# PKU-EPIC/GAPartNet

Hardware: AMD Instinct MI355X
Metric: point-clouds/sec (20k pts, train step) (higher is better)
Workload: dtype f32

## Files before the change

gapartnet_amd/csrc/bn.hip:

```cpp
#include <cstdlib>

#include "bn_stats.h"
#include "gpn_common.h"

namespace {

typedef float f32x4 __attribute__((ext_vector_type(4)));
constexpr int kThreads = 256;
constexpr int kMaxBlocks = 128;


template <int T>
__device__ __forceinline__ double column_total(const double (*red)[T][4], int q, int c, int C4, int R, int part, int P) {
  double acc = 0.0;
  const int cc4 = c >> 2, j = c & 3;
  for (int rr = part; rr < R; rr += P) acc += red[q][rr * C4 + cc4][j];
  for (int off = P >> 1; off >= 1; off >>= 1) acc += __shfl_down(acc, off, P);
  return acc;
}

__host__ __device__ __forceinline__ int sub_lanes(int pairs, int T) {
  int P = 16;
  while (P > 1 && pairs * P > T) P >>= 1;
  return P;
// ... 302 lines not shown
        if (res) v += rv[k];
        if (relu) {
#pragma unroll
          for (int j = 0; j < 4; ++j) v[j] = v[j] > 0.f ? v[j] : 0.f;
        }
        reinterpret_cast<f32x4*>(y)[tt] = v;
      }
      c4 += step;
      c4 = c4 >= C4 ? c4 - C4 : c4;
    }
    t += U * stride;
    if (t >= total4) break;
#pragma unroll
    for (int k = 0; k < U; ++k) {
      const int64_t tt = t + k * stride;
      if (tt < total4) {
        xv[k] = reinterpret_cast<const f32x4*>(x)[tt];
        if (res) rv[k] = reinterpret_cast<const f32x4*>(res)[tt];
      }
    }
  }
}

template <bool FIXED>
__global__ __launch_bounds__(kApplyThreads) void bn_apply_bwd_fold_kernel(gpn::BnBwdPtrs pa, gpn::BnBwdPtrs pb, int blocks, int64_t total4,
                                                                         int C4, float inv_n, int relu, int training,
                                                                         const int64_t* __restrict__ n_dev) {
  if (n_dev) {
    const int64_t N = gpn::live_rows(n_dev, total4 / C4);
    total4 = N * C4;
    inv_n = 1.0f / (float)N;
    if (N == 0) {
      if (blockIdx.x == 0) {
        const gpn::BnBwdPtrs& q = blockIdx.y ? pb : pa;
        for (int c = threadIdx.x; c < C4 * 4; c += kApplyThreads) q.dbias[c] = 0.f, q.dweight[c] = 0.f;
      }
      return;
    }
  }
  const gpn::BnBwdPtrs& pp = blockIdx.y ? pb : pa;
  const float* __restrict__ x = pp.x;
  const float* __restrict__ y = pp.y;
  const float* __restrict__ dy = pp.dy;
  const void* __restrict__ partial = pp.partial;
  const float* __restrict__ mean = pp.mean;
  const float* __restrict__ invstd = pp.invstd;
  const float* __restrict__ weight = pp.weight;
  float* __restrict__ dx = pp.dx;
  float* __restrict__ dres = pp.dres;
  float* __restrict__ dweight = pp.dweight;
  float* __restrict__ dbias = pp.dbias;
  __shared__ double red[2][FIXED ? 1 : kApplyThreads][4];
  __shared__ unsigned long long words[FIXED ? 4 : 1][FIXED ? kFoldMaxC : 1];
  __shared__ double sums[2][kFoldMaxC];
  __shared__ __attribute__((aligned(16))) float stat[5][kFoldMaxC];
  constexpr int U = kApplyBatch;
  const int C = C4 * 4;
  const int64_t stride = (int64_t)gridDim.x * kApplyThreads;
  const int step = (int)(stride % C4);
  int64_t t = (int64_t)blockIdx.x * kApplyThreads + threadIdx.x;
  int c4 = (int)(t % C4);
  f32x4 gv[U], yv[U], xv[U];
#pragma unroll
  for (int k = 0; k < U; ++k) {
    const int64_t tt = t + k * stride;
    if (tt < total4) {
      gv[k] = reinterpret_cast<const f32x4*>(dy)[tt];
      if (relu) yv[k] = reinterpret_cast<const f32x4*>(y)[tt];
      if (training) xv[k] = reinterpret_cast<const f32x4*>(x)[tt];
    }
  }
  if constexpr (FIXED)
    fold_fixed<true>(static_cast<const unsigned long long*>(partial), C, blocks, reinterpret_cast<unsigned long long (*)[kFoldMaxC]>(&words[0][0]), sums);
  else
    fold_partials(static_cast<const double*>(partial), blocks, C4, reinterpret_cast<double (*)[kApplyThreads][4]>(&red[0][0][0]), sums);
  for (int c = threadIdx.x; c < C; c += kApplyThreads) {
    const float db = (float)sums[0][c], dw = (float)sums[1][c];
    stat[0][c] = db;
    stat[1][c] = dw;
    stat[2][c] = mean[c];
    stat[3][c] = invstd[c];
    stat[4][c] = weight[c];
    if (blockIdx.x == 0) {
      dbias[c] = db;
      dweight[c] = dw;
    }
  }
  __syncthreads();
  while (true) {
#pragma unroll
    for (int k = 0; k < U; ++k) {
      const int64_t tt = t + k * stride;
      if (tt < total4) {
        const f32x4 is = reinterpret_cast<const f32x4*>(stat[3])[c4], w = reinterpret_cast<const f32x4*>(stat[4])[c4];
        f32x4 g = gv[k];
        if (relu) {
#pragma unroll
          for (int j = 0; j < 4; ++j) g[j] = yv[k][j] > 0.f ? g[j] : 0.f;
        }
        if (dres) reinterpret_cast<f32x4*>(dres)[tt] = g;
        f32x4 v = g;
        if (training) {
          const f32x4 db = reinterpret_cast<const f32x4*>(stat[0])[c4], dw = reinterpret_cast<const f32x4*>(stat[1])[c4];
          const f32x4 mu = reinterpret_cast<const f32x4*>(stat[2])[c4];
          const f32x4 xhat = (xv[k] - mu) * is;
          v = g - db * inv_n - xhat * (dw * inv_n);
        }
        reinterpret_cast<f32x4*>(dx)[tt] = v * is * w;
      }
      c4 += step;
      c4 = c4 >= C4 ? c4 - C4 : c4;
    }
    t += U * stride;
    if (t >= total4) break;
#pragma unroll
    for (int k = 0; k < U; ++k) {
      const int64_t tt = t + k * stride;
      if (tt < total4) {
        gv[k] = reinterpret_cast<const f32x4*>(dy)[tt];
        if (relu) yv[k] = reinterpret_cast<const f32x4*>(y)[tt];
        if (training) xv[k] = reinterpret_cast<const f32x4*>(x)[tt];
      }
    }
  }
}

constexpr int kSmallRows = 1024;

template <int CG, int T>
__device__ __forceinline__ void column_sum8(double (&v)[8], double (*scratch)[CG][8] ) {
  constexpr int W = T / 64;
#pragma unroll
  for (int off = 32; off >= CG; off >>= 1) {
#pragma unroll
    for (int q = 0; q < 8; ++q) v[q] += __shfl_down(v[q], off, 64);
  }
  if ((threadIdx.x & 63) < CG) {
#pragma unroll
    for (int q = 0; q < 8; ++q) scratch[threadIdx.x >> 6][threadIdx.x & 63][q] = v[q];
  }
  __syncthreads();
  const int cg = threadIdx.x % CG;
#pragma unroll
// ... 302 lines not shown
}

bool gpn::bn_two_pass(int64_t N, int C) { return N >= 1 && C % 4 == 0 && C <= kFoldMaxC; }

int gpn::bn_fwd_train_fused(const gpn::BnFwdPtrs& p, const gpn::BnFwdPtrs* twin, int64_t N, int C, float eps, float momentum,
                            int relu, hipStream_t stream, const gpn::DevRows& rows) {
  for (const gpn::BnFwdPtrs* q : {&p, twin}) {
    if (!q) continue;
    GPN_CHECK_ARG(q->x && q->weight && q->bias && q->y && q->mean && q->invstd && q->partial);
    GPN_CHECK_ARG((q->running_mean == nullptr) == (q->running_var == nullptr));
  }
  GPN_CHECK_ARG(gpn::bn_two_pass(N, C));
  GPN_CHECK_ARG(!twin || (twin->res == nullptr) == (p.res == nullptr));
  const int64_t total4 = N * (C / 4);
  gpn::ProfScope prof(GPN_K_BN, stream, 0.0, 4.0 * (double)N * C * (p.res ? 3 : 2) * (twin ? 2 : 1), rows.dev, N);
  const int64_t Np = gpn::plan_rows(N, rows);
  hipLaunchKernelGGL(bn_apply_fwd_fold_kernel<true>, dim3(fold_grid(Np * (C / 4)), twin ? 2 : 1), dim3(kApplyThreads), 0, stream, p,
                     twin ? *twin : p, gpn::stat_slot_count(Np), N, total4, C / 4, eps, momentum, relu, rows.dev);
  GPN_CHECK_LAUNCH();
  return GPN_OK;
}

int gpn::bn_bwd_fused(const gpn::BnBwdPtrs& p, const gpn::BnBwdPtrs* twin, int64_t N, int C, int relu, int training,
                      hipStream_t stream, const gpn::DevRows& rows) {
  for (const gpn::BnBwdPtrs* q : {&p, twin}) {
    if (!q) continue;
    GPN_CHECK_ARG(q->x && q->dy && q->weight && q->mean && q->invstd && q->dx && q->dweight && q->dbias && q->partial && (q->y || !relu));
  }
  GPN_CHECK_ARG(gpn::bn_two_pass(N, C));
  GPN_CHECK_ARG(!twin || (twin->dres == nullptr) == (p.dres == nullptr));
  const int64_t total4 = N * (C / 4);
  gpn::ProfScope prof(GPN_K_BN, stream, 0.0, 4.0 * (double)N * C * (4 + (p.dres ? 1 : 0)) * (twin ? 2 : 1), rows.dev, N);
  const int64_t Np = gpn::plan_rows(N, rows);
  hipLaunchKernelGGL(bn_apply_bwd_fold_kernel<true>, dim3(fold_grid(Np * (C / 4)), twin ? 2 : 1), dim3(kApplyThreads), 0, stream, p,
                     twin ? *twin : p, gpn::stat_slot_count(Np), total4, C / 4, 1.0f / (float)N, relu, training, rows.dev);
  GPN_CHECK_LAUNCH();
  return GPN_OK;
}
```

gapartnet_amd/csrc/gpn_common.h:

```cpp
#pragma once
#include <cstdlib>
#include <cstring>
#include <hip/hip_runtime.h>

#include <cstdint>
#include <cstdio>

#include "../../include/gpn.h"

namespace gpn {

void set_error(const char* fmt, ...);

struct ProfScope {
  int id;
  hipStream_t stream;
  hipEvent_t start = nullptr;
  int64_t tag = 0;
  ProfScope(int kernel_id, hipStream_t s, double flops, double bytes, int64_t tag = 0);
  ProfScope(int kernel_id, hipStream_t s, double flops, double bytes, const int64_t* rows_dev, int64_t bound, int64_t tag = 0);
  ~ProfScope();
};
inline int64_t prof_shape_tag(int K, int64_t n_dst, int cin, int cout, bool twin) {
  return ((int64_t)(twin ? 1 : 0) << 62) | ((int64_t)(K & 63) << 48) | ((int64_t)((cin / 16) & 255) << 40) |
// ... 45 lines not shown
  bool ok() const { return used <= cap && (base != nullptr || used == 0); }
};

constexpr int kStatSlots = 32;
inline int stat_slot_count(int64_t rows) {
  const int64_t tiles = (rows + 15) / 16;
  int s = 1;
  while (s < kStatSlots && tiles > 64 * (int64_t)s) s *= 2;
  return s;
}
struct ConvAffine {
  const float* mean = nullptr;
  const float* var = nullptr;
  const float* weight = nullptr;
  const float* bias = nullptr;
  const float* res = nullptr;
  float eps = 0.f;
  int relu = 0;
};
struct ConvTwin {
  const float* in = nullptr;
  const float* packed = nullptr;
  float* out = nullptr;
  unsigned long long* slab = nullptr;
  const float* x = nullptr;
  const float* y = nullptr;
  const float* mean = nullptr;
  const float* invstd = nullptr;
  ConvAffine ep;
};
struct ConvStats {
  unsigned long long* slab = nullptr;
  int slot_mask = kStatSlots - 1;
  const float* x = nullptr;
  const float* y = nullptr;
  const float* mean = nullptr;
  const float* invstd = nullptr;
  int relu = 0;
  ConvAffine ep;
  ConvTwin twin;
};
#ifdef __HIPCC__
struct AffineCol {
  float mu, is, w, b;
};
__device__ __forceinline__ AffineCol affine_col(const ConvAffine& ep, uint32_t col) {
  return AffineCol{ep.mean[col], 1.0f / sqrtf(ep.var[col] + ep.eps), ep.weight[col], ep.bias[col]};
}
__device__ __forceinline__ float affine_apply(const ConvAffine& ep, const AffineCol& c, float v, uint32_t e) {
  v = (v - c.mu) * c.is * c.w + c.b;
  if (ep.res) v += ep.res[e];
  if (ep.relu) v = v > 0.f ? v : 0.f;
  return v;
}
#endif
struct BnFwdPtrs {
  const float* x = nullptr;
  const float* res = nullptr;
  const void* partial = nullptr;
  const float* weight = nullptr;
  const float* bias = nullptr;
// ... 52 lines not shown
};
struct WgradSets {
  int n = 0;
  WgradSet s[kWgradSets];
};
struct WgradReduceJob {
  const float* partial;
  float* dW;
  int64_t elems;
  int S, K, cin, cout, oki, few;
};
int wgrad_slices(int K, int cin, int cout, int64_t n_dst);
int wgrad_contract(const WgradSets& sets, int K, int64_t n_dst, int cin, int cout, int S, hipStream_t stream,
                   const int64_t* n_dst_dev = nullptr);
WgradReduceJob wgrad_reduce_job(const float* partial, int S, int K, int cin, int cout, int flags, float* dW);
int wgrad_reduce_many(const WgradReduceJob* jobs, int n, hipStream_t stream);
int rulebook_level_counts_dev(const int32_t* indices, int64_t n_max, const int64_t* n_dev, int64_t batch_size,
                              const int64_t* max_coord_dev, int n_levels, int64_t* counts, void* ws, size_t ws_bytes,
                              hipStream_t stream);
bool bn_two_pass(int64_t N, int C);
int bn_fwd_train_fused(const BnFwdPtrs& p, const BnFwdPtrs* twin, int64_t N, int C, float eps, float momentum, int relu,
                       hipStream_t stream, const DevRows& rows = DevRows());
int bn_bwd_fused(const BnBwdPtrs& p, const BnBwdPtrs* twin, int64_t N, int C, int relu, int training, hipStream_t stream,
                 const DevRows& rows = DevRows());
int bn_fwd_train_rows(const float* x, const float* res, const float* weight, const float* bias, int64_t N, const DevRows& rows,
                      int C, float eps, float momentum, int relu, float* y, float* mean, float* invstd, float* running_mean,
                      float* running_var, void* ws, size_t ws_bytes, hipStream_t stream);
int bn_fwd_eval_rows(const float* x, const float* res, const float* weight, const float* bias, const float* mean,
                     const float* invstd, int64_t N, const DevRows& rows, int C, int relu, float* y, hipStream_t stream);
int bn_fwd_eval_running(const BnFwdPtrs& pa, const BnFwdPtrs* pb, int64_t N, const DevRows& rows, int C, float eps, int relu,
                        hipStream_t stream);
int bn_bwd_rows(const float* x, const float* y, const float* dy, const float* weight, const float* mean, const float* invstd,
                int64_t N, const DevRows& rows, int C, int relu, int training, float* dx, float* dres, float* dweight,
                float* dbias, void* ws, size_t ws_bytes, hipStream_t stream);

}

#define GPN_CHECK_ARG(cond)                                                     \
  do {                                                                          \
    if (!(cond)) {                                                              \
      gpn::set_error("%s: bad argument: %s", __func__, #cond);                  \
      return GPN_ERR_ARG;                                                       \
    }                                                                           \
  } while (0)

#define GPN_CHECK_HIP(expr)                                                     \
  do {                                                                          \
// ... 24 lines not shown
```

gapartnet_amd/csrc/net.hip:

```cpp
#include <unistd.h>

#include <cstdlib>

#include <algorithm>
#include <atomic>
#include <condition_variable>
#include <mutex>
#include <string>
#include <thread>
#include <vector>

#include "gpn_common.h"
#include "spconv_pack.h"

namespace {

constexpr int kThreads = 256;

std::atomic<int> g_bn_fusion{1};

struct ConcatPtrs {
  const float4* a;
  const float4* b;
  float4* dst;
// ... 683 lines not shown
    if (rc) return rc;
  }
  const Need need = workspace_need(ops, n_ops, nets[0].slots, rbs, nets[0].convs);
  const size_t per_net = need.tmp + need.packed + need.stats;
  const size_t total_need = n_nets * per_net + need.op + n_nets * need.wgrad;
  if (!ws || ws_bytes < total_need) {
    gpn::set_error("%s: workspace too small (%zu needed, %zu given)", who, total_need, ws_bytes);
    return GPN_ERR_WS;
  }
  char* base = static_cast<char*>(ws);
  float* tmp[2] = {reinterpret_cast<float*>(base), reinterpret_cast<float*>(base + per_net)};
  void* op_ws = base + n_nets * per_net;
  const size_t op_ws_bytes = need.op;
  void* wgrad_ws = base + n_nets * per_net + need.op;
  const size_t wgrad_ws_bytes = ws_bytes - (n_nets * per_net + need.op);
  std::vector<const float*> packed_of[2];
  for (int t = 0; t < n_nets; ++t) {
    rc = pack_program(ops, n_ops, rbs, nets[t].convs, true, base + t * per_net + need.tmp, packed_of[t], stream);
    if (rc) return rc;
  }
  std::vector<unsigned long long*> bn_slab[2];
  for (int t = 0; t < n_nets; ++t) bn_slab[t].assign(n_ops, nullptr);
  std::vector<int> fused_by(n_ops, -1);
  std::vector<char> sums_done(n_ops, 0);
  if (g_bn_fusion.load(std::memory_order_relaxed)) {
    std::vector<int> first_reader(n_slots, -1), producer(n_slots, -1);
    for (int i = n_ops - 1; i >= 0; --i) {
      first_reader[ops[i].src0] = i;
      if (ops[i].src1 >= 0) first_reader[ops[i].src1] = i;
      producer[ops[i].dst] = i;
    }
    size_t off = 0;
    for (int i = 0; i < n_ops; ++i) {
      if (ops[i].kind != GPN_NET_CONV) continue;
      const int j = producer[ops[i].src0];
      if (j < 0 || ops[j].kind != GPN_NET_BN || first_reader[ops[i].src0] != i) continue;
      if (ops[i].src0 == 0 && !need_input_grad) continue;
      const gpn_net_rulebook_t& rb = rbs[ops[i].rulebook];
      const gpn_net_conv_t& cv = nets[0].convs[ops[i].param];
      const gpn_net_slot_t& in_slot = nets[0].slots[ops[i].src0];
      if (!gpn::bn_two_pass(plan_of(in_slot), cv.cin) ||
          !gpn::spconv_fwd_route(rb.K, rb.n_src, cv.cout, cv.cin, dev_rows(in_slot)).sums)
        continue;
      for (int t = 0; t < n_nets; ++t)
        bn_slab[t][j] = reinterpret_cast<unsigned long long*>(base + t * per_net + need.tmp + need.packed + off);
      off += gpn::stat_slab_bytes(cv.cin);
      fused_by[i] = j;
// ... 65 lines not shown
      }
      if (op.src0 != 0 || need_input_grad) {
        for (int t = 0; t < n_nets; ++t)
          if (!nets[t].slots[op.src0].grad || !rb.nbr_t) {
            gpn::set_error("%s: op %d: null gradient buffer / transposed table", who, i);
            return GPN_ERR_ARG;
          }
        gpn::ConvStats st;
        if (pair) {
          st.twin.in = nets[1].slots[op.dst].grad;
          st.twin.packed = packed_of[1][i];
          st.twin.out = nets[1].slots[op.src0].grad;
        }
        if (fused_by[i] >= 0) {
          const gpn_net_op_t& bo = ops[fused_by[i]];
          const gpn_net_bn_t& bn = nets[0].bns[bo.param];
          st.slab = bn_slab[0][fused_by[i]];
          st.slot_mask = gpn::stat_slot_count(plan_of(s0)) - 1;
          st.x = nets[0].slots[bo.src0].data;
          st.y = s0.data;
          st.mean = training ? bn.save_mean : bn.running_mean;
          st.invstd = bn.save_invstd;
          st.relu = (bo.flags & GPN_NET_RELU) ? 1 : 0;
          if (pair) {
            const gpn_net_bn_t& bn1 = nets[1].bns[bo.param];
            st.twin.slab = bn_slab[1][fused_by[i]];
            st.twin.x = nets[1].slots[bo.src0].data;
            st.twin.y = nets[1].slots[op.src0].data;
            st.twin.mean = training ? bn1.save_mean : bn1.running_mean;
            st.twin.invstd = bn1.save_invstd;
          }
          sums_done[fused_by[i]] = 1;
        }
        rc = gpn::spconv_fwd_into(d.grad, packed_of[0][i], rb.nbr_t, rb.nbr_t_p, rb.perm_t, rb.K, rb.n_src, cv.cout, cv.cin, s0.grad,
                                  s0.grad_state ? 1 : 0, st, op_ws, op_ws_bytes, stream, dev_rows(s0));
        if (rc) return rc;
        for (int t = 0; t < n_nets; ++t) nets[t].slots[op.src0].grad_state = 1;
      }
    } else if (op.kind == GPN_NET_BN) {
      const int relu = (op.flags & GPN_NET_RELU) ? 1 : 0;
      gpn::BnBwdPtrs pp[2];
      GradTarget tr[2] = {{nullptr, false}, {nullptr, false}};
      for (int t = 0; t < n_nets; ++t) {
        const gpn_net_bn_t& bn = nets[t].bns[op.param];
        gpn_net_slot_t& ts0 = nets[t].slots[op.src0];
        if (!ts0.grad || !bn.dweight || !bn.dbias) {
          gpn::set_error("%s: op %d: null gradient buffer", who, i);
          return GPN_ERR_ARG;
        }
        GradTarget tx = grad_target(ts0, tmp[t]);
        if (tx.staged) {
          gpn::set_error("%s: op %d: BatchNorm input consumed twice is not supported", who, i);
          return GPN_ERR_ARG;
        }
        if (op.src1 >= 0 && (op.src1 != 0 || need_input_grad)) {
          if (!nets[t].slots[op.src1].grad) {
            gpn::set_error("%s: op %d: null residual gradient buffer", who, i);
            return GPN_ERR_ARG;
          }
          tr[t] = grad_target(nets[t].slots[op.src1], tmp[t]);
        }
        pp[t].x = ts0.data, pp[t].y = nets[t].slots[op.dst].data, pp[t].dy = nets[t].slots[op.dst].grad;
        pp[t].partial = bn_slab[t][i];
        pp[t].mean = training ? bn.save_mean : bn.running_mean;
        pp[t].invstd = bn.save_invstd, pp[t].weight = bn.weight;
        pp[t].dx = tx.ptr, pp[t].dres = tr[t].ptr, pp[t].dweight = bn.dweight, pp[t].dbias = bn.dbias;
      }
      const gpn_net_bn_t& bn0 = nets[0].bns[op.param];
      if (sums_done[i] && pair) {
        rc = gpn::bn_bwd_fused(pp[0], &pp[1], s0.rows, bn0.C, relu, training ? 1 : 0, stream, dev_rows(s0));
      } else {
        for (int t = 0; t < n_nets && rc == GPN_OK; ++t) {
          if (sums_done[i])
            rc = gpn::bn_bwd_fused(pp[t], nullptr, s0.rows, bn0.C, relu, training ? 1 : 0, stream, dev_rows(s0));
          else
            rc = gpn::bn_bwd_rows(pp[t].x, pp[t].y, pp[t].dy, pp[t].weight, pp[t].mean, pp[t].invstd, s0.rows, dev_rows(s0), bn0.C, relu,
                                  training ? 1 : 0, pp[t].dx, pp[t].dres, pp[t].dweight, pp[t].dbias, op_ws, op_ws_bytes, stream);
        }
      }
      if (rc) return rc;
      for (int t = 0; t < n_nets; ++t) {
        nets[t].slots[op.src0].grad_state = 1;
        if (pp[t].dres) {
          rc = commit(nets[t].slots[op.src1], tr[t], stream);
          if (rc) return rc;
        }
      }
    } else {
      gpn_net_slot_t& s1 = nets[0].slots[op.src1];
      for (int t = 0; t < n_nets; ++t)
        if (!nets[t].slots[op.src0].grad || !nets[t].slots[op.src1].grad) {
          gpn::set_error("%s: op %d: null gradient buffer", who, i);
          return GPN_ERR_ARG;
        }
      SplitPtrs sa{(const float4*)d.grad, (float4*)s0.grad, (float4*)s1.grad}, sb = sa;
      if (pair)
        sb = SplitPtrs{(const float4*)nets[1].slots[op.dst].grad, (float4*)nets[1].slots[op.src0].grad,
                       (float4*)nets[1].slots[op.src1].grad};
      hipLaunchKernelGGL(split_kernel, dim3(grid_for(plan_of(d) * (d.channels / 4)), n_nets), dim3(kThreads), 0, stream, sa, sb, d.rows,
                         s0.channels / 4, s1.channels / 4, s0.grad_state, s1.grad_state, d.rows_dev);
      GPN_CHECK_LAUNCH();
      for (int t = 0; t < n_nets; ++t) nets[t].slots[op.src0].grad_state = nets[t].slots[op.src1].grad_state = 1;
    }
  }
  std::string worker_err;
// ... 219 lines not shown
```

gapartnet_amd/csrc/spconv_fwd.hip:

```cpp
#include <algorithm>
#include <atomic>
#include <cstdlib>

#include "bn_stats.h"
#include "spconv_dispatch.h"

namespace {

typedef float f32x4 __attribute__((ext_vector_type(4)));

template <int NTW, int CW>
struct FwdCfg {
  static constexpr int SLAB_V4 = CW * NTW * 64;
  static constexpr int D = (CW * NTW >= 8) ? 2 : 4;
  static constexpr size_t lds_bytes = (size_t)2 * SLAB_V4 * 16;
};

struct StageCursor {
  int k, ch;
  __device__ __forceinline__ void advance(int nch) {
    ++ch;
    if (ch == nch) { ch = 0; ++k; }
  }
};
// ... 204 lines not shown
}

int launch_lockstep(const FwdPlan& p, const gpn::ConvCall& c) {
#define GPN_X(v) if (p.ntw == v) return dispatch_cw<v>(p, c);
  GPN_LOCKSTEP_NTW(GPN_X)
#undef GPN_X
  return gpn::conv_no_kernel("lock-step", c);
}

#ifndef GPN_ABL
#define GPN_ABL 0
#endif
#ifndef GPN_DIRECT_D
#define GPN_DIRECT_D 4
#endif
template <int KT, int CB, bool DEV, bool EP>
__global__ __launch_bounds__(256) void spconv_fwd_direct_kernel(const float* __restrict__ in, const float* __restrict__ packed,
                                                                const int32_t* __restrict__ nbr, int64_t n_dst, int nt_total,
                                                                int64_t units, size_t packed_bytes,
                                                                const int32_t* __restrict__ perm, int accumulate,
                                                                gpn::ConvStats stats, float* __restrict__ out,
                                                                const int64_t* __restrict__ n_dev) {
  if (blockIdx.y) {
    in = stats.twin.in, packed = stats.twin.packed, out = stats.twin.out;
    stats.slab = stats.twin.slab, stats.x = stats.twin.x, stats.y = stats.twin.y, stats.mean = stats.twin.mean,
    stats.invstd = stats.twin.invstd;
    if constexpr (EP) {
      const float eps = stats.ep.eps;
      const int relu = stats.ep.relu;
      stats.ep = stats.twin.ep, stats.ep.eps = eps, stats.ep.relu = relu;
    }
  }
  constexpr int S = KT * CB;
  constexpr int D = S >= GPN_DIRECT_D ? GPN_DIRECT_D : S;
  const int lane = threadIdx.x & 63, wave = threadIdx.x >> 6;
  const int i16 = lane & 15, g = lane >> 4;
  if constexpr (DEV) {
    n_dst = gpn::live_rows(n_dev, n_dst);
    units = ((n_dst + 15) >> 4) * nt_total;
  }
  auto run_unit = [&](const int64_t unit) {
  const int64_t tile = unit / nt_total;
  const int nt = (int)(unit - tile * nt_total);
  const int cin = CB * 16, cout = nt_total * 16;
  const __amdgpu_buffer_rsrc_t in_rsrc = __builtin_amdgcn_make_buffer_rsrc(const_cast<float*>(in), 0, 0x7fffffff, 0x00020000);
  const __amdgpu_buffer_rsrc_t nbr_rsrc =
      __builtin_amdgcn_make_buffer_rsrc(const_cast<int32_t*>(nbr), 0, 0x7fffffff, 0x00020000);
// ... 80 lines not shown
#endif
      }
      acc += part;
    } else {
#pragma unroll
      for (int cb = 0; cb < CB; ++cb) {
        const int s = tap * CB + cb;
        if (s + D < S) issue(s + D, s % D);
      }
    }
    if (tap + DI < KT) ireg[tap % DI] = load_idx(tap + DI);
    asm volatile("" ::: "memory");
  }
  const bool st_fwd = stats.slab != nullptr && stats.x == nullptr;
  double s0 = 0.0, s1 = 0.0;
  gpn::AffineCol ac;
  if constexpr (EP) ac = gpn::affine_col(stats.ep, col);
#pragma unroll
  for (int r = 0; r < 4; ++r) {
    const int64_t row = row0 + 4 * g + r;
    if (row < n_dst) {
      const uint32_t e = (uint32_t)orow[r] * (uint32_t)cout + col;
      float v = acc[r];
      if (accumulate) v += out[e];
      if constexpr (EP) v = gpn::affine_apply(stats.ep, ac, v, e);
      out[e] = v;
      if (st_fwd) {
        s0 += (double)v;
        s1 += (double)v * (double)v;
      } else if (st_bwd) {
        const float gm = (stats.relu && !(by[r] > 0.f)) ? 0.f : v;
        s0 += (double)gm;
        s1 += (double)gm * (double)((bx[r] - mu) * is);
      }
    }
  }
  if (st_fwd) gpn::stat_add<false>(stats.slab, cout, (int)(tile & stats.slot_mask), (int)col, g, gpn::stat_reduce_g(s0), gpn::stat_reduce_g(s1));
  else if (st_bwd) gpn::stat_add<true>(stats.slab, cout, (int)(tile & stats.slot_mask), (int)col, g, gpn::stat_reduce_g(s0), gpn::stat_reduce_g(s1));
  };
  if constexpr (!DEV) {
    const int64_t wg = (int64_t)(blockIdx.x & 7) * (gridDim.x >> 3) + (blockIdx.x >> 3);
    const int64_t unit = wg * 4 + wave;
    if (unit >= units) return;
    run_unit(unit);
  } else {
    const int64_t per8 = (((units + 3) >> 2) + 7) >> 3;
    for (int64_t wj = blockIdx.x >> 3; wj < per8; wj += gridDim.x >> 3) {
      const int64_t unit = ((int64_t)(blockIdx.x & 7) * per8 + wj) * 4 + wave;
      if (unit < units) run_unit(unit);
    }
  }
}

#ifndef GPN_SPLIT_TRACE
#define GPN_SPLIT_TRACE 0
#endif
#if GPN_SPLIT_TRACE
__device__ unsigned long long* g_split_trace = nullptr;
#endif
template <int KT, int CB, int SP, bool DEV>
__global__ __launch_bounds__(256) void spconv_fwd_split_kernel(const float* __restrict__ in, const float* __restrict__ packed,
                                                               const int32_t* __restrict__ nbr, int64_t n_dst, int nt_total,
                                                               int64_t units, size_t packed_bytes,
                                                               const int32_t* __restrict__ perm, int accumulate,
                                                               gpn::ConvStats stats, float* __restrict__ out,
                                                               const int64_t* __restrict__ n_dev) {
  constexpr int TP = (KT + SP - 1) / SP;
  constexpr int S = TP * CB;
  constexpr int D = S >= GPN_DIRECT_D ? GPN_DIRECT_D : S;
  constexpr int UPW = 4 / SP;
  __shared__ f32x4 red[4][64];
  if (blockIdx.y) {
    in = stats.twin.in, packed = stats.twin.packed, out = stats.twin.out;
    stats.slab = stats.twin.slab, stats.x = stats.twin.x, stats.y = stats.twin.y, stats.mean = stats.twin.mean,
    stats.invstd = stats.twin.invstd;
  }
  const int lane = threadIdx.x & 63, wave = threadIdx.x >> 6;
  const int i16 = lane & 15, g = lane >> 4;
  if constexpr (DEV) {
    n_dst = gpn::live_rows(n_dev, n_dst);
    units = ((n_dst + 15) >> 4) * nt_total;
  }
  auto run_wg = [&](const int64_t wg, const bool more) {
#if GPN_SPLIT_TRACE
  const unsigned long long tr0 = wall_clock64();
#endif
  const int64_t unit = wg * UPW + wave / SP;
  const int part = wave % SP;
  const int tap0 = part * TP;
  const bool active = unit < units;
  const int64_t tile = active ? unit / nt_total : 0;
  const int nt = active ? (int)(unit - tile * nt_total) : 0;
  const int cin = CB * 16, cout = nt_total * 16;
  const __amdgpu_buffer_rsrc_t in_rsrc = __builtin_amdgcn_make_buffer_rsrc(const_cast<float*>(in), 0, 0x7fffffff, 0x00020000);
  const __amdgpu_buffer_rsrc_t nbr_rsrc =
      __builtin_amdgcn_make_buffer_rsrc(const_cast<int32_t*>(nbr), 0, 0x7fffffff, 0x00020000);
// ... 85 lines not shown
    asm volatile("" ::: "memory");
  }
#if GPN_SPLIT_TRACE
  __builtin_amdgcn_s_waitcnt(0);
  const unsigned long long tr2 = wall_clock64();
#endif
  if (part != 0) red[wave][lane] = acc;
  __syncthreads();
#if GPN_SPLIT_TRACE
  const unsigned long long tr3 = wall_clock64();
#endif
  if (part == 0 && active) {
#pragma unroll
  for (int q = 1; q < SP; ++q) acc += red[wave + q][lane];

  const bool st_fwd = stats.slab != nullptr && stats.x == nullptr;
  double s0 = 0.0, s1 = 0.0;
#pragma unroll
  for (int r = 0; r < 4; ++r) {
    const int64_t row = row0 + 4 * g + r;
    if (row < n_dst) {
      const uint32_t e = (uint32_t)orow[r] * (uint32_t)cout + col;
      float v = acc[r];
      if (accumulate) v += out[e];
      out[e] = v;
      if (st_fwd) {
        s0 += (double)v;
        s1 += (double)v * (double)v;
      } else if (st_bwd) {
        const float gm = (stats.relu && !(by[r] > 0.f)) ? 0.f : v;
        s0 += (double)gm;
        s1 += (double)gm * (double)((bx[r] - mu) * is);
      }
    }
  }
  if (st_fwd) gpn::stat_add<false>(stats.slab, cout, (int)(tile & stats.slot_mask), (int)col, g, gpn::stat_reduce_g(s0), gpn::stat_reduce_g(s1));
  else if (st_bwd) gpn::stat_add<true>(stats.slab, cout, (int)(tile & stats.slot_mask), (int)col, g, gpn::stat_reduce_g(s0), gpn::stat_reduce_g(s1));
  }
#if GPN_SPLIT_TRACE
  if (g_split_trace && blockIdx.y == 0 && active) {
    __builtin_amdgcn_s_waitcnt(0);
    const unsigned long long tr4 = wall_clock64();
    if (lane == 0) {
      unsigned long long* t = g_split_trace + ((size_t)unit * SP + part) * 10;
      t[0] = tr0, t[1] = tr1, t[2] = tr1, t[3] = tr2, t[4] = tr3, t[5] = tr4, t[6] = (unsigned long long)TP;
      t[7] = (unsigned long long)__builtin_amdgcn_s_getreg((31 << 11) | 4);
      t[8] = (unsigned long long)__builtin_amdgcn_s_getreg((31 << 11) | 20);
      t[9] = (unsigned long long)blockIdx.x;
    }
  }
#endif
  if (more) __syncthreads();
  };
// ... 220 lines not shown
```

gapartnet_amd/csrc/spconv_msplit.hip:

```cpp
#include <algorithm>
#include <atomic>
#include <cstdlib>

#include "bn_stats.h"
#include "spconv_dispatch.h"

namespace {

typedef float f32x4 __attribute__((ext_vector_type(4)));
constexpr int kMaxTaps = 27;

#ifndef GPN_MSPLIT_TRACE
#define GPN_MSPLIT_TRACE 0
#endif
#if GPN_MSPLIT_TRACE
__device__ unsigned long long* g_msplit_trace = nullptr;
#endif
#ifndef GPN_MSPLIT_ABL
#define GPN_MSPLIT_ABL 0
#endif
#ifndef GPN_MSPLIT_OPERAND_REGS
#define GPN_MSPLIT_OPERAND_REGS 48
#endif

// ... 5 lines not shown
  st = st < 1 ? 1 : st;
  while (st * CB < 3) ++st;
  st = st > 4 ? 4 : st;
  return st > max_tp ? max_tp : st;
}

#ifndef GPN_MSPLIT_OCC_HINTS
#define GPN_MSPLIT_OCC_HINTS 1
#endif
constexpr int ms_occ(int CB, int NT, int SP, bool DEV) {
  if (!GPN_MSPLIT_OCC_HINTS || DEV) return 1;
  if (SP == 4 && CB == 3 && NT == 3) return 5;
  return 1;
}
#define GPN_MSPLIT_OCC __attribute__((amdgpu_waves_per_eu(ms_occ(CB, NT, SP, DEV))))
template <int CB, int NT, int SP, bool DEV, bool EP>
__global__ __launch_bounds__(SP * 64) GPN_MSPLIT_OCC void spconv_msplit_kernel(const float* __restrict__ in, const float* __restrict__ packed,
                                                                const int32_t* __restrict__ nbr, const int32_t* __restrict__ perm,
                                                                int K, int64_t n_dst, int n_tiles, int n_units, int nt_total,
                                                                int col_groups, size_t packed_bytes, int accumulate,
                                                                gpn::ConvStats stats, float* __restrict__ out,
                                                                const int64_t* __restrict__ n_dev) {
  if (blockIdx.y) {
    in = stats.twin.in, packed = stats.twin.packed, out = stats.twin.out;
    stats.slab = stats.twin.slab, stats.x = stats.twin.x, stats.y = stats.twin.y, stats.mean = stats.twin.mean,
    stats.invstd = stats.twin.invstd;
    if constexpr (EP) {
      const float eps = stats.ep.eps;
      const int relu = stats.ep.relu;
      stats.ep = stats.twin.ep, stats.ep.eps = eps, stats.ep.relu = relu;
    }
  }
  constexpr int MAXTP = (kMaxTaps + SP - 1) / SP;
  constexpr int NI = (MAXTP + 3) / 4;
  constexpr int NF = (NT + SP - 1) / SP;
  constexpr uint32_t kOob = 0x80000000u;
  __shared__ uint32_t slab[SP][MAXTP + 1][16];
  __shared__ f32x4 red[SP][NT][64];

  const int lane = threadIdx.x & 63, wave = threadIdx.x >> 6;
  const int i16 = lane & 15, g = lane >> 4;
  if constexpr (DEV) {
    n_dst = gpn::live_rows(n_dev, n_dst);
    n_tiles = (int)((n_dst + 15) >> 4);
    n_units = n_tiles * col_groups;
  }
  const int TP = (K + SP - 1) / SP;
// ... 164 lines not shown
#pragma unroll
  for (int nt = 0; nt < NT; ++nt) red[wave][nt][lane] = acc[nt];
  __syncthreads();
#if GPN_MSPLIT_TRACE
  const unsigned long long tr3 = wall_clock64();
#endif
  const bool st_fwd = stats.slab != nullptr && stats.x == nullptr;
#pragma unroll
  for (int f = 0; f < NF; ++f) {
    const int nt = wave + f * SP;
    if (nt < NT) {
      f32x4 v4 = red[0][nt][lane];
#pragma unroll
      for (int q = 1; q < SP; ++q) v4 += red[q][nt][lane];
      const uint32_t col = (uint32_t)((nt0 + nt) * 16 + i16);
      double s0 = 0.0, s1 = 0.0;
      gpn::AffineCol ac;
      if constexpr (EP) ac = gpn::affine_col(stats.ep, col);
#pragma unroll
      for (int r = 0; r < 4; ++r) {
        if ((int64_t)tile * 16 + 4 * g + r < n_dst) {
          const uint32_t e = (uint32_t)orow[r] * (uint32_t)cout + col;
          float v = v4[r];
          if (accumulate) v += out[e];
          if constexpr (EP) v = gpn::affine_apply(stats.ep, ac, v, e);
          out[e] = v;
          if (st_fwd) {
            s0 += (double)v;
            s1 += (double)v * (double)v;
          } else if (st_bwd) {
            const float gm = (stats.relu && !(by[f][r] > 0.f)) ? 0.f : v;
            s0 += (double)gm;
            s1 += (double)gm * (double)((bx[f][r] - bmu[f]) * bis[f]);
          }
        }
      }
      if (st_fwd) gpn::stat_add<false>(stats.slab, cout, (int)(tile & stats.slot_mask), (int)col, g, gpn::stat_reduce_g(s0), gpn::stat_reduce_g(s1));
      else if (st_bwd) gpn::stat_add<true>(stats.slab, cout, (int)(tile & stats.slot_mask), (int)col, g, gpn::stat_reduce_g(s0), gpn::stat_reduce_g(s1));
    }
  }
#if GPN_MSPLIT_TRACE
  if (g_msplit_trace && blockIdx.y == 0) {
    __builtin_amdgcn_s_waitcnt(0);
    const unsigned long long tr4 = wall_clock64();
    if (lane == 0) {
      unsigned long long* t = g_msplit_trace + ((size_t)unit * SP + wave) * 10;
      t[0] = tr0, t[1] = tr1, t[2] = tr1b, t[3] = tr2, t[4] = tr3, t[5] = tr4, t[6] = tr_taps;
      t[7] = (unsigned long long)__builtin_amdgcn_s_getreg((31 << 11) | 4);
      t[8] = (unsigned long long)__builtin_amdgcn_s_getreg((31 << 11) | 20);
      t[9] = (unsigned long long)blockIdx.x;
    }
  }
#endif
  if (more) __syncthreads();
// ... 114 lines not shown
```

gapartnet_amd/csrc/spconv_tiles.hip:

```cpp
#include <algorithm>
#include <atomic>
#include <cstdlib>

#include "bn_stats.h"
#include "spconv_dispatch.h"

namespace {

typedef float f32x4 __attribute__((ext_vector_type(4)));
typedef __bf16 bf16x8 __attribute__((ext_vector_type(8)));
constexpr int kMaxTaps = 27;

__device__ __forceinline__ void split_bf16x3(const f32x4 a0, const f32x4 a1, bf16x8& hi, bf16x8& mid, bf16x8& lo) {
  const float x[8] = {a0.x, a0.y, a0.z, a0.w, a1.x, a1.y, a1.z, a1.w};
#pragma unroll
  for (int i = 0; i < 8; ++i) {
    const __bf16 h = (__bf16)x[i];
    const float r1 = x[i] - (float)h;
    const __bf16 m = (__bf16)r1;
    hi[i] = h, mid[i] = m, lo[i] = (__bf16)(r1 - (float)m);
  }
}

#ifndef GPN_TILES_ABL
// ... 6 lines not shown
#ifndef GPN_TILES_TRACE
#define GPN_TILES_TRACE 0
#endif
#if GPN_TILES_TRACE
__device__ unsigned long long* g_tiles_trace = nullptr;
#endif

using gpn::static_for;

constexpr int cfg_slots(int CB, int R, int NT) {
  const int regs_per_tap = CB * (R + NT) * 4 + ((GPN_TILES_ABL & 16) ? (CB / 2) * NT * 4 : 0);
  const int S = GPN_TILES_OPERAND_REGS / regs_per_tap;
  return S < 2 ? 2 : (S > 6 ? 6 : S);
}

template <int CB, int NT, int R, bool DEV, bool EP>
__global__ __launch_bounds__(256) void spconv_tiles_kernel(const float* __restrict__ in, const float* __restrict__ packed,
                                                           const int32_t* __restrict__ nbr, const int32_t* __restrict__ perm,
                                                           int K, int64_t n_dst, int n_tiles, int n_units, int nt_total,
                                                           int col_groups, size_t packed_bytes, int accumulate,
                                                           gpn::ConvStats stats, float* __restrict__ out,
                                                           const int64_t* __restrict__ n_dev) {
  if (blockIdx.y) {
    in = stats.twin.in, packed = stats.twin.packed, out = stats.twin.out;
    stats.slab = stats.twin.slab, stats.x = stats.twin.x, stats.y = stats.twin.y, stats.mean = stats.twin.mean,
    stats.invstd = stats.twin.invstd;
    if constexpr (EP) {
      const float eps = stats.ep.eps;
      const int relu = stats.ep.relu;
      stats.ep = stats.twin.ep, stats.ep.eps = eps, stats.ep.relu = relu;
    }
  }
  constexpr int RW = R * 16;
  constexpr int TPI = 64 / RW;
  constexpr int NI = (kMaxTaps + TPI - 1) / TPI;
  constexpr uint32_t kOob = 0x80000000u;
  __shared__ uint32_t slab[4][kMaxTaps + 1][RW];

  const int lane = threadIdx.x & 63, wave = threadIdx.x >> 6;
  const int i16 = lane & 15, g = lane >> 4;
  if constexpr (DEV) {
    n_dst = gpn::live_rows(n_dev, n_dst);
    n_tiles = (int)((n_dst + 15) >> 4);
    n_units = ((n_tiles + R - 1) / R) * col_groups;
  }
  auto run_unit = [&](const int unit) {
#if GPN_TILES_TRACE
// ... 211 lines not shown
    if (decltype(i)::value < remaining) consume(i);
  });

#if GPN_TILES_TRACE
  __builtin_amdgcn_s_waitcnt(0);
  const unsigned long long tr2 = wall_clock64();
#endif
  const bool st_fwd = (GPN_TILES_ABL & 8) == 0 && stats.slab != nullptr && stats.x == nullptr;
#pragma unroll
  for (int t = 0; t < R; ++t) {
    const int tile = tile0 + t;
    if (tile < n_tiles) {
#pragma unroll
      for (int nt = 0; nt < NT; ++nt) {
        const uint32_t col = (uint32_t)((nt0 + nt) * 16 + i16);
        double s0 = 0.0, s1 = 0.0;
        gpn::AffineCol ac;
        if constexpr (EP) ac = gpn::affine_col(stats.ep, col);
#pragma unroll
        for (int r = 0; r < 4; ++r) {
          if ((int64_t)tile * 16 + 4 * g + r < n_dst) {
            const uint32_t e = (uint32_t)orow[t][r] * (uint32_t)cout + col;
            float v = acc[t][nt][r];
            if (accumulate) v += out[e];
            if constexpr (EP) v = gpn::affine_apply(stats.ep, ac, v, e);
            out[e] = v;
            if (st_fwd) {
              s0 += (double)v;
              s1 += (double)v * (double)v;
            } else if (st_bwd) {
              const float gm = (stats.relu && !(by[t][nt][r] > 0.f)) ? 0.f : v;
              s0 += (double)gm;
              s1 += (double)gm * (double)((bx[t][nt][r] - bmu[nt]) * bis[nt]);
            }
          }
        }
        if (st_fwd) gpn::stat_add<false>(stats.slab, cout, (int)(tile & stats.slot_mask), (int)col, g, gpn::stat_reduce_g(s0), gpn::stat_reduce_g(s1));
        else if (st_bwd) gpn::stat_add<true>(stats.slab, cout, (int)(tile & stats.slot_mask), (int)col, g, gpn::stat_reduce_g(s0), gpn::stat_reduce_g(s1));
      }
    }
  }
#if GPN_TILES_TRACE
  if (g_tiles_trace && blockIdx.y == 0) {
    __builtin_amdgcn_s_waitcnt(0);
    const unsigned long long tr3 = wall_clock64();
    if (lane == 0) {
      unsigned long long* t = g_tiles_trace + (size_t)unit * 8;
      t[0] = tr0, t[1] = tr1, t[2] = tr2, t[3] = tr3, t[4] = tr_taps;
      t[5] = (unsigned long long)__builtin_amdgcn_s_getreg((31 << 11) | 4);
      t[6] = (unsigned long long)__builtin_amdgcn_s_getreg((31 << 11) | 20);
      t[7] = (unsigned long long)blockIdx.x;
    }
  }
#endif
// ... 91 lines not shown
```

Baseline: 1044.

## Store relu-masked gradient from conv epilogue and redirect residual grad buffer

The dgrad conv epilogue now writes the relu-masked gradient directly, so the following BN backward kernel can skip loading y for the mask. When a residual gradient buffer is not shared with other slots, the conv reads the old gradient and writes the sum into the residual's gradient buffer. The BN backward then reads dy from that buffer and skips writing dres, which removes a full-tensor store and the later commit. This adds aliasing checks and more template variants, and it changes which buffer holds the gradient, so correctness depends on the overlap analysis.

```diff
diff --git a/gapartnet_amd/csrc/bn.hip b/gapartnet_amd/csrc/bn.hip
--- a/gapartnet_amd/csrc/bn.hip
+++ b/gapartnet_amd/csrc/bn.hip
@@ -1,4 +1,5 @@
 #include <cstdlib>
+#include <type_traits>
 
 #include "bn_stats.h"
 #include "gpn_common.h"
@@ -348,7 +349,7 @@
   }
 }
 
-template <bool FIXED>
+template <bool FIXED, bool MASKED = false, bool DRES = true>
 __global__ __launch_bounds__(kApplyThreads) void bn_apply_bwd_fold_kernel(gpn::BnBwdPtrs pa, gpn::BnBwdPtrs pb, int blocks, int64_t total4,
                                                                          int C4, float inv_n, int relu, int training,
                                                                          const int64_t* __restrict__ n_dev) {
@@ -386,13 +387,15 @@
   const int step = (int)(stride % C4);
   int64_t t = (int64_t)blockIdx.x * kApplyThreads + threadIdx.x;
   int c4 = (int)(t % C4);
+  static_assert(FIXED || !MASKED, "only a conv launch's epilogue masks the gradient it stores");
+  const bool select = relu && !MASKED;
   f32x4 gv[U], yv[U], xv[U];
 #pragma unroll
   for (int k = 0; k < U; ++k) {
     const int64_t tt = t + k * stride;
     if (tt < total4) {
       gv[k] = reinterpret_cast<const f32x4*>(dy)[tt];
-      if (relu) yv[k] = reinterpret_cast<const f32x4*>(y)[tt];
+      if (select) yv[k] = reinterpret_cast<const f32x4*>(y)[tt];
       if (training) xv[k] = reinterpret_cast<const f32x4*>(x)[tt];
     }
   }
@@ -420,11 +423,11 @@
       if (tt < total4) {
         const f32x4 is = reinterpret_cast<const f32x4*>(stat[3])[c4], w = reinterpret_cast<const f32x4*>(stat[4])[c4];
         f32x4 g = gv[k];
-        if (relu) {
+        if (select) {
 #pragma unroll
           for (int j = 0; j < 4; ++j) g[j] = yv[k][j] > 0.f ? g[j] : 0.f;
         }
-        if (dres) reinterpret_cast<f32x4*>(dres)[tt] = g;
+        if (DRES && dres) reinterpret_cast<f32x4*>(dres)[tt] = g;
         f32x4 v = g;
         if (training) {
           const f32x4 db = reinterpret_cast<const f32x4*>(stat[0])[c4], dw = reinterpret_cast<const f32x4*>(stat[1])[c4];
@@ -444,7 +447,7 @@
       const int64_t tt = t + k * stride;
       if (tt < total4) {
         gv[k] = reinterpret_cast<const f32x4*>(dy)[tt];
-        if (relu) yv[k] = reinterpret_cast<const f32x4*>(y)[tt];
+        if (select) yv[k] = reinterpret_cast<const f32x4*>(y)[tt];
         if (training) xv[k] = reinterpret_cast<const f32x4*>(x)[tt];
       }
     }
@@ -793,18 +796,27 @@
 }
 
 int gpn::bn_bwd_fused(const gpn::BnBwdPtrs& p, const gpn::BnBwdPtrs* twin, int64_t N, int C, int relu, int training,
-                      hipStream_t stream, const gpn::DevRows& rows) {
+                      hipStream_t stream, const gpn::DevRows& rows, bool dy_masked) {
   for (const gpn::BnBwdPtrs* q : {&p, twin}) {
     if (!q) continue;
-    GPN_CHECK_ARG(q->x && q->dy && q->weight && q->mean && q->invstd && q->dx && q->dweight && q->dbias && q->partial && (q->y || !relu));
+    GPN_CHECK_ARG(q->x && q->dy && q->weight && q->mean && q->invstd && q->dx && q->dweight && q->dbias && q->partial &&
+                  (q->y || !relu || dy_masked));
   }
   GPN_CHECK_ARG(gpn::bn_two_pass(N, C));
   GPN_CHECK_ARG(!twin || (twin->dres == nullptr) == (p.dres == nullptr));
   const int64_t total4 = N * (C / 4);
-  gpn::ProfScope prof(GPN_K_BN, stream, 0.0, 4.0 * (double)N * C * (4 + (p.dres ? 1 : 0)) * (twin ? 2 : 1), rows.dev, N);
+  const bool masked = relu && dy_masked;
+  gpn::ProfScope prof(GPN_K_BN, stream, 0.0, 4.0 * (double)N * C * (4 - (masked ? 1 : 0) + (p.dres ? 1 : 0)) * (twin ? 2 : 1), rows.dev, N);
   const int64_t Np = gpn::plan_rows(N, rows);
-  hipLaunchKernelGGL(bn_apply_bwd_fold_kernel<true>, dim3(fold_grid(Np * (C / 4)), twin ? 2 : 1), dim3(kApplyThreads), 0, stream, p,
-                     twin ? *twin : p, gpn::stat_slot_count(Np), total4, C / 4, 1.0f / (float)N, relu, training, rows.dev);
+  const dim3 grid(fold_grid(Np * (C / 4)), twin ? 2 : 1);
+  auto launch = [&](auto m, auto r) {
+    hipLaunchKernelGGL((bn_apply_bwd_fold_kernel<true, decltype(m)::value, decltype(r)::value>), grid, dim3(kApplyThreads), 0, stream, p,
+                       twin ? *twin : p, gpn::stat_slot_count(Np), total4, C / 4, 1.0f / (float)N, relu, training, rows.dev);
+  };
+  if (masked && p.dres) launch(std::true_type(), std::true_type());
+  else if (masked) launch(std::true_type(), std::false_type());
+  else if (p.dres) launch(std::false_type(), std::true_type());
+  else launch(std::false_type(), std::false_type());
   GPN_CHECK_LAUNCH();
   return GPN_OK;
 }
diff --git a/gapartnet_amd/csrc/gpn_common.h b/gapartnet_amd/csrc/gpn_common.h
--- a/gapartnet_amd/csrc/gpn_common.h
+++ b/gapartnet_amd/csrc/gpn_common.h
@@ -91,6 +91,7 @@
   const float* in = nullptr;
   const float* packed = nullptr;
   float* out = nullptr;
+  const float* acc = nullptr;
   unsigned long long* slab = nullptr;
   const float* x = nullptr;
   const float* y = nullptr;
@@ -106,6 +107,7 @@
   const float* mean = nullptr;
   const float* invstd = nullptr;
   int relu = 0;
+  const float* acc = nullptr;
   ConvAffine ep;
   ConvTwin twin;
 };
@@ -204,7 +206,7 @@
 int bn_fwd_train_fused(const BnFwdPtrs& p, const BnFwdPtrs* twin, int64_t N, int C, float eps, float momentum, int relu,
                        hipStream_t stream, const DevRows& rows = DevRows());
 int bn_bwd_fused(const BnBwdPtrs& p, const BnBwdPtrs* twin, int64_t N, int C, int relu, int training, hipStream_t stream,
-                 const DevRows& rows = DevRows());
+                 const DevRows& rows = DevRows(), bool dy_masked = false);
 int bn_fwd_train_rows(const float* x, const float* res, const float* weight, const float* bias, int64_t N, const DevRows& rows,
                       int C, float eps, float momentum, int relu, float* y, float* mean, float* invstd, float* running_mean,
                       float* running_var, void* ws, size_t ws_bytes, hipStream_t stream);
diff --git a/gapartnet_amd/csrc/net.hip b/gapartnet_amd/csrc/net.hip
--- a/gapartnet_amd/csrc/net.hip
+++ b/gapartnet_amd/csrc/net.hip
@@ -729,7 +729,34 @@
   std::vector<unsigned long long*> bn_slab[2];
   for (int t = 0; t < n_nets; ++t) bn_slab[t].assign(n_ops, nullptr);
   std::vector<int> fused_by(n_ops, -1);
-  std::vector<char> sums_done(n_ops, 0);
+  std::vector<char> sums_done(n_ops, 0), redirected(n_ops, 0);
+  auto grad_distinct = [&](int r) {
+    for (int t = 0; t < n_nets; ++t) {
+      const gpn_net_slot_t& a = nets[t].slots[r];
+      const char* a0 = reinterpret_cast<const char*>(a.grad);
+      const char* a1 = a0 + (size_t)a.rows * a.channels * sizeof(float);
+      for (int u = 0; u < n_nets; ++u)
+        for (int q = 0; q < n_slots; ++q) {
+          const gpn_net_slot_t& b = nets[u].slots[q];
+          if ((u == t && q == r) || !b.grad) continue;
+          const char* b0 = reinterpret_cast<const char*>(b.grad);
+          if (a0 < b0 + (size_t)b.rows * b.channels * sizeof(float) && b0 < a1) return false;
+        }
+    }
+    return true;
+  };
+  auto can_redirect = [&](int i, int j) {
+    const int r = ops[j].src1, s = ops[i].src0;
+    if (r <= 0 || r == s) return false;
+    for (int k = j + 1; k < i; ++k)
+      if (ops[k].src0 == r || ops[k].src1 == r) return false;
+    for (int t = 0; t < n_nets; ++t) {
+      const gpn_net_slot_t &R = nets[t].slots[r], &S = nets[t].slots[s];
+      if (!R.grad || R.grad_state) return false;
+      if (R.rows != S.rows || R.channels != S.channels || R.rows_dev != S.rows_dev || R.rows_plan != S.rows_plan) return false;
+    }
+    return grad_distinct(r);
+  };
   if (g_bn_fusion.load(std::memory_order_relaxed)) {
     std::vector<int> first_reader(n_slots, -1), producer(n_slots, -1);
     for (int i = n_ops - 1; i >= 0; --i) {
@@ -841,6 +868,11 @@
           st.mean = training ? bn.save_mean : bn.running_mean;
           st.invstd = bn.save_invstd;
           st.relu = (bo.flags & GPN_NET_RELU) ? 1 : 0;
+          if (can_redirect(i, fused_by[i])) {
+            redirected[fused_by[i]] = 1;
+            st.acc = s0.grad;
+            if (pair) st.twin.acc = st.twin.out, st.twin.out = nets[1].slots[bo.src1].grad;
+          }
           if (pair) {
             const gpn_net_bn_t& bn1 = nets[1].bns[bo.param];
             st.twin.slab = bn_slab[1][fused_by[i]];
@@ -851,7 +883,8 @@
           }
           sums_done[fused_by[i]] = 1;
         }
-        rc = gpn::spconv_fwd_into(d.grad, packed_of[0][i], rb.nbr_t, rb.nbr_t_p, rb.perm_t, rb.K, rb.n_src, cv.cout, cv.cin, s0.grad,
+        float* dgrad_out = st.acc ? nets[0].slots[ops[fused_by[i]].src1].grad : s0.grad;
+        rc = gpn::spconv_fwd_into(d.grad, packed_of[0][i], rb.nbr_t, rb.nbr_t_p, rb.perm_t, rb.K, rb.n_src, cv.cout, cv.cin, dgrad_out,
                                   s0.grad_state ? 1 : 0, st, op_ws, op_ws_bytes, stream, dev_rows(s0));
         if (rc) return rc;
         for (int t = 0; t < n_nets; ++t) nets[t].slots[op.src0].grad_state = 1;
@@ -872,14 +905,15 @@
           gpn::set_error("%s: op %d: BatchNorm input consumed twice is not supported", who, i);
           return GPN_ERR_ARG;
         }
-        if (op.src1 >= 0 && (op.src1 != 0 || need_input_grad)) {
+        if (op.src1 >= 0 && (op.src1 != 0 || need_input_grad) && !redirected[i]) {
           if (!nets[t].slots[op.src1].grad) {
             gpn::set_error("%s: op %d: null residual gradient buffer", who, i);
             return GPN_ERR_ARG;
           }
           tr[t] = grad_target(nets[t].slots[op.src1], tmp[t]);
         }
-        pp[t].x = ts0.data, pp[t].y = nets[t].slots[op.dst].data, pp[t].dy = nets[t].slots[op.dst].grad;
+        pp[t].x = ts0.data, pp[t].y = nets[t].slots[op.dst].data;
+        pp[t].dy = redirected[i] ? nets[t].slots[op.src1].grad : nets[t].slots[op.dst].grad;
         pp[t].partial = bn_slab[t][i];
         pp[t].mean = training ? bn.save_mean : bn.running_mean;
         pp[t].invstd = bn.save_invstd, pp[t].weight = bn.weight;
@@ -887,11 +921,11 @@
       }
       const gpn_net_bn_t& bn0 = nets[0].bns[op.param];
       if (sums_done[i] && pair) {
-        rc = gpn::bn_bwd_fused(pp[0], &pp[1], s0.rows, bn0.C, relu, training ? 1 : 0, stream, dev_rows(s0));
+        rc = gpn::bn_bwd_fused(pp[0], &pp[1], s0.rows, bn0.C, relu, training ? 1 : 0, stream, dev_rows(s0), true);
       } else {
         for (int t = 0; t < n_nets && rc == GPN_OK; ++t) {
           if (sums_done[i])
-            rc = gpn::bn_bwd_fused(pp[t], nullptr, s0.rows, bn0.C, relu, training ? 1 : 0, stream, dev_rows(s0));
+            rc = gpn::bn_bwd_fused(pp[t], nullptr, s0.rows, bn0.C, relu, training ? 1 : 0, stream, dev_rows(s0), true);
           else
             rc = gpn::bn_bwd_rows(pp[t].x, pp[t].y, pp[t].dy, pp[t].weight, pp[t].mean, pp[t].invstd, s0.rows, dev_rows(s0), bn0.C, relu,
                                   training ? 1 : 0, pp[t].dx, pp[t].dres, pp[t].dweight, pp[t].dbias, op_ws, op_ws_bytes, stream);
@@ -900,6 +934,7 @@
       if (rc) return rc;
       for (int t = 0; t < n_nets; ++t) {
         nets[t].slots[op.src0].grad_state = 1;
+        if (redirected[i]) nets[t].slots[op.src1].grad_state = 1;
         if (pp[t].dres) {
           rc = commit(nets[t].slots[op.src1], tr[t], stream);
           if (rc) return rc;
diff --git a/gapartnet_amd/csrc/spconv_fwd.hip b/gapartnet_amd/csrc/spconv_fwd.hip
--- a/gapartnet_amd/csrc/spconv_fwd.hip
+++ b/gapartnet_amd/csrc/spconv_fwd.hip
@@ -250,7 +250,7 @@
                                                                 gpn::ConvStats stats, float* __restrict__ out,
                                                                 const int64_t* __restrict__ n_dev) {
   if (blockIdx.y) {
-    in = stats.twin.in, packed = stats.twin.packed, out = stats.twin.out;
+    in = stats.twin.in, packed = stats.twin.packed, out = stats.twin.out, stats.acc = stats.twin.acc;
     stats.slab = stats.twin.slab, stats.x = stats.twin.x, stats.y = stats.twin.y, stats.mean = stats.twin.mean,
     stats.invstd = stats.twin.invstd;
     if constexpr (EP) {
@@ -377,14 +377,14 @@
     if (row < n_dst) {
       const uint32_t e = (uint32_t)orow[r] * (uint32_t)cout + col;
       float v = acc[r];
-      if (accumulate) v += out[e];
+      if (accumulate) v += (stats.acc ? stats.acc : out)[e];
       if constexpr (EP) v = gpn::affine_apply(stats.ep, ac, v, e);
-      out[e] = v;
+      const float gm = (st_bwd && stats.relu && !(by[r] > 0.f)) ? 0.f : v;
+      out[e] = gm;
       if (st_fwd) {
         s0 += (double)v;
         s1 += (double)v * (double)v;
       } else if (st_bwd) {
-        const float gm = (stats.relu && !(by[r] > 0.f)) ? 0.f : v;
         s0 += (double)gm;
         s1 += (double)gm * (double)((bx[r] - mu) * is);
       }
@@ -426,7 +426,7 @@
   constexpr int UPW = 4 / SP;
   __shared__ f32x4 red[4][64];
   if (blockIdx.y) {
-    in = stats.twin.in, packed = stats.twin.packed, out = stats.twin.out;
+    in = stats.twin.in, packed = stats.twin.packed, out = stats.twin.out, stats.acc = stats.twin.acc;
     stats.slab = stats.twin.slab, stats.x = stats.twin.x, stats.y = stats.twin.y, stats.mean = stats.twin.mean,
     stats.invstd = stats.twin.invstd;
   }
@@ -558,13 +558,13 @@
     if (row < n_dst) {
       const uint32_t e = (uint32_t)orow[r] * (uint32_t)cout + col;
       float v = acc[r];
-      if (accumulate) v += out[e];
-      out[e] = v;
+      if (accumulate) v += (stats.acc ? stats.acc : out)[e];
+      const float gm = (st_bwd && stats.relu && !(by[r] > 0.f)) ? 0.f : v;
+      out[e] = gm;
       if (st_fwd) {
         s0 += (double)v;
         s1 += (double)v * (double)v;
       } else if (st_bwd) {
-        const float gm = (stats.relu && !(by[r] > 0.f)) ? 0.f : v;
         s0 += (double)gm;
         s1 += (double)gm * (double)((bx[r] - mu) * is);
       }
diff --git a/gapartnet_amd/csrc/spconv_msplit.hip b/gapartnet_amd/csrc/spconv_msplit.hip
--- a/gapartnet_amd/csrc/spconv_msplit.hip
+++ b/gapartnet_amd/csrc/spconv_msplit.hip
@@ -51,7 +51,7 @@
                                                                 gpn::ConvStats stats, float* __restrict__ out,
                                                                 const int64_t* __restrict__ n_dev) {
   if (blockIdx.y) {
-    in = stats.twin.in, packed = stats.twin.packed, out = stats.twin.out;
+    in = stats.twin.in, packed = stats.twin.packed, out = stats.twin.out, stats.acc = stats.twin.acc;
     stats.slab = stats.twin.slab, stats.x = stats.twin.x, stats.y = stats.twin.y, stats.mean = stats.twin.mean,
     stats.invstd = stats.twin.invstd;
     if constexpr (EP) {
@@ -262,14 +262,14 @@
         if ((int64_t)tile * 16 + 4 * g + r < n_dst) {
           const uint32_t e = (uint32_t)orow[r] * (uint32_t)cout + col;
           float v = v4[r];
-          if (accumulate) v += out[e];
+          if (accumulate) v += (stats.acc ? stats.acc : out)[e];
           if constexpr (EP) v = gpn::affine_apply(stats.ep, ac, v, e);
-          out[e] = v;
+          const float gm = (st_bwd && stats.relu && !(by[f][r] > 0.f)) ? 0.f : v;
+          out[e] = gm;
           if (st_fwd) {
             s0 += (double)v;
             s1 += (double)v * (double)v;
           } else if (st_bwd) {
-            const float gm = (stats.relu && !(by[f][r] > 0.f)) ? 0.f : v;
             s0 += (double)gm;
             s1 += (double)gm * (double)((bx[f][r] - bmu[f]) * bis[f]);
           }
diff --git a/gapartnet_amd/csrc/spconv_tiles.hip b/gapartnet_amd/csrc/spconv_tiles.hip
--- a/gapartnet_amd/csrc/spconv_tiles.hip
+++ b/gapartnet_amd/csrc/spconv_tiles.hip
@@ -52,7 +52,7 @@
                                                            gpn::ConvStats stats, float* __restrict__ out,
                                                            const int64_t* __restrict__ n_dev) {
   if (blockIdx.y) {
-    in = stats.twin.in, packed = stats.twin.packed, out = stats.twin.out;
+    in = stats.twin.in, packed = stats.twin.packed, out = stats.twin.out, stats.acc = stats.twin.acc;
     stats.slab = stats.twin.slab, stats.x = stats.twin.x, stats.y = stats.twin.y, stats.mean = stats.twin.mean,
     stats.invstd = stats.twin.invstd;
     if constexpr (EP) {
@@ -310,14 +310,14 @@
           if ((int64_t)tile * 16 + 4 * g + r < n_dst) {
             const uint32_t e = (uint32_t)orow[t][r] * (uint32_t)cout + col;
             float v = acc[t][nt][r];
-            if (accumulate) v += out[e];
+            if (accumulate) v += (stats.acc ? stats.acc : out)[e];
             if constexpr (EP) v = gpn::affine_apply(stats.ep, ac, v, e);
-            out[e] = v;
+            const float gm = (st_bwd && stats.relu && !(by[t][nt][r] > 0.f)) ? 0.f : v;
+            out[e] = gm;
             if (st_fwd) {
               s0 += (double)v;
               s1 += (double)v * (double)v;
             } else if (st_bwd) {
-              const float gm = (stats.relu && !(by[t][nt][r] > 0.f)) ? 0.f : v;
               s0 += (double)gm;
               s1 += (double)gm * (double)((bx[t][nt][r] - bmu[nt]) * bis[nt]);
             }
```

New measurement: 1048, median of 5. No clear change (+0.4%).
